# Gabisanth/MaximumAreaCoverageOptimization.jl

Measured on AMD Instinct MI355X. Metric: MADS objective evals/sec (N UAVs × M fire cells), 1/2/4/8 MI355X, higher is better.
Workload: dtype f64

## Files before the change

### maximumareacoverageoptimization.jl_amd/csrc/k_prep.h

```cpp
#pragma once

#include <hip/hip_runtime.h>
#include <stdint.h>

#include "predicate.h"
#include "k_common.h"

#pragma clang fp contract(off)

namespace mac {


struct PenArgs {
    const double* rmax;
    const double* prev;
    const double* dlimT;
    const double* dlim;
    double tan_half_fov;
};

__device__ __forceinline__ double pen_threshold(const PenArgs& pa, int i)
{
    if (!pa.prev) return 0.0;
    return pa.dlimT ? pa.dlimT[i] : dlim_threshold(pa.dlim[i]);
// ... 69 lines not shown
struct CandSrc {
    const double* cands;
    int ldc;
    const uint32_t* keysP;
    const float* keysT;
    int ldk;
    const double* xinc;
    const int* rp;
    const int* cp;
    uint64_t state;
    int64_t b;
    int k0;
    int np;
    const MadsState* mst;
    const int16_t* ltri;
    double delta;
    int route_five;
    __device__ __forceinline__ bool resolve(bool any_poll = false)
    {
        if (!mst) return true;
        const int e = mst->ell;
        if (e < 0 || (!any_poll && mst->skip)) return false;
        b = (int64_t)1 << e;
        return true;
    }
    __host__ __device__ __forceinline__ int polled(int N) const { return np ? np : 3 * N; }
    __device__ __forceinline__ double entry(int n, int r, int c) const
    {
        if (ltri) return r < c ? 0.0 : delta * (double)ltri[(int64_t)r * (r + 1) / 2 + c];
        return ltmads_entry(state, n, b, r, c);
    }
    __device__ __forceinline__ double get_full(int kl, int v, int N) const
    {
        if (cands) return cands[(int64_t)kl * ldc + v];
        const int n = 3 * N;
        const int k = kl + k0;
        const int kk = k < n ? k : k - n;
        const double d = entry(n, rp[v], cp[kk]);
        return k < n ? xinc[v] + d : xinc[v] - d;
    }
    __device__ __forceinline__ double get(int kl, int v, int N) const
    {
        if (cands) return cands[(int64_t)kl * ldc + v];
        const int n = polled(N);
        const int k = kl + k0;
        const int kk = k < n ? k : k - n;
        const bool held = v >= n;
        const double xv = xinc[v];
        const double d = entry(n, rp[held ? 0 : v], cp[kk]);
        const double moved = k < n ? xv + d : xv - d;
        return held ? xv : moved;
    }
};

#ifndef MAC_PREP_C
#define MAC_PREP_C 8
#endif
constexpr int kPrepC = MAC_PREP_C;
constexpr int kPrepU = 512;

static_assert(kPrepC % 4 == 0 && 32 % kPrepC == 0 && kPrepC <= 64,
              "MAC_PREP_C must divide 32 and be a multiple of 4");
__host__ __device__ inline int keys_ld(int K) { return (K + 31) & ~31; }

struct PrepArgs {
    CandSrc src;
    int N, K;
    PenArgs pa;
    double penalty;
    double* vp;
    int pair;
    int nchain;
    int skip_failed;
    int xbase;
    int4* prec;
    Grid g;
    uint32_t* keysP;
    float* keysT;
    int ldk;
    double4* pd;
    uint8_t* dead8;
    MadsState* mst_w;
    unsigned long long* feas;
    int* lreset;
    const uint8_t* mask8;
};

template <int NC, class Cand>
__device__ __forceinline__ uint32_t prep_masked(const uint8_t* mask8, int K, Cand cand)
{
    uint32_t m = 0u;
    if (mask8) {
#pragma unroll
        for (int c = 0; c < NC; ++c) {
            const int k = cand(c);
            if (k < K && mask8[k] == 0) m |= 1u << c;
        }
    }
    return m;
}

constexpr int kPrepCX = 6;

constexpr uint32_t kKeyEsc = 0x200u << 22;
__device__ __forceinline__ bool key_int(double v, double b, double lim, int& d)
{
    const double f = v - b;
    if (!(f >= -lim && f <= lim)) return false;
    d = (int)f;
    return (double)d == f && __builtin_bit_cast(uint64_t, b + (double)d) == __builtin_bit_cast(uint64_t, v);
}
__device__ __forceinline__ uint32_t key_pack(int dx, int dy, int dr)
{
    return ((uint32_t)dx & 0x7FFu) | (((uint32_t)dy & 0x7FFu) << 11) | (((uint32_t)dr & 0x3FFu) << 22);
}
__device__ __forceinline__ void key_unpack(uint32_t p, float& x, float& y, float& r)
{
    x = (float)((int)(p << 21) >> 21);
    y = (float)((int)(p << 10) >> 21);
    r = (float)((int)p >> 22);
}

__device__ __forceinline__ bool partial_range(double a, double b, double m, double g0, double invS,
                                              int n, int& lo, int& hi)
{
    const double ulo = (a - g0) * invS;
    const double uhi = (b - g0) * invS;
    const double err = (m + __builtin_fabs(g0)) * invS * 1e-14 + 1e-9;
    const double flo = __builtin_floor(ulo - err);
    const double fhi = __builtin_floor(uhi + err);
    if (!(flo == flo) || !(fhi == fhi)) { lo = 0; hi = n - 1; return true; }
    if (fhi < 0.0 || flo > (double)(n - 1)) return false;
    lo = flo < 0.0 ? 0 : (int)flo;
    hi = fhi > (double)(n - 1) ? n - 1 : (int)fhi;
    return true;
}

__host__ __device__ inline int range_shift(int n)
{
    int s = 0;
    while (((n - 1) >> s) > 0xFFFE) ++s;
    return s;
}
__device__ __forceinline__ uint32_t range_pack(bool any, int lo, int hi, int s)
{
    return any ? (uint32_t)(lo >> s) | ((uint32_t)(hi >> s) << 16) : 0xFFFFu;
}
__device__ __forceinline__ void range_unpack(uint32_t lo16, uint32_t hi16, int s, int n, int& lo, int& hi)
{
    lo = (int)(lo16 << s);
    hi = min((int)(((hi16 + 1) << s) - 1), n - 1);
}

#ifdef MAC_DIAG
__device__ uint64_t g_diag_prep[64 * 16];
#define MAC_PREP_STAMP_T(q, t) if (threadIdx.x == (t) && cw < 64 && (q) < 16) g_diag_prep[16 * cw + (q)] = __builtin_amdgcn_s_memrealtime()
#else
#define MAC_PREP_STAMP_T(q, t)
#endif
#define MAC_PREP_STAMP(q) MAC_PREP_STAMP_T(q, 0)

__device__ __forceinline__ void lds_barrier()
{
    asm volatile("s_waitcnt lgkmcnt(0)\n\ts_barrier" ::: "memory");
}

template <int PC>
struct PrepLds {
    double term[PC][kPrepU + 2];
    int wbad[kPrepU / kWave][PC];
    uint32_t wbadm[kPrepU / kWave];
    int wrej[kPrepU / kWave];
    double dred[kPrepU / kWave][4];
};

template <bool kMat, int PC>
__device__ __forceinline__ void prep_block(const PrepArgs& a, int cw, unsigned char* lds)
{
    constexpr int NC = PC;
    PrepLds<NC>& L = *reinterpret_cast<PrepLds<NC>*>(lds);
    auto& term = L.term;
    auto& wbad = L.wbad;
    auto& wbadm = L.wbadm;
    auto& wrej = L.wrej;
    auto& dred = L.dred;
    const int N = a.N, K = a.K;
    const int u = threadIdx.x, lane = u & (kWave - 1), wid = u / kWave;
    const int k0 = cw * PC;
    const int np = a.src.polled(N);
    auto cand = [&](int c) { return a.pair ? (c < 4 ? 4 * cw + c : np + 4 * cw + c - 4) : k0 + c; };
    const bool obj = a.vp != nullptr;
    const PenArgs& pa = a.pa;
    MAC_PREP_STAMP(0);
    double acc = 0.0;
    bool bad = false;
    uint32_t mdead = 0u;
    if constexpr (!kMat) mdead = prep_masked<NC>(obj ? a.mask8 : nullptr, K, cand);
    const bool masked = !kMat && a.mask8 != nullptr;
    const bool excl = obj && (pa.prev || masked) && (a.prec || a.pd) && a.skip_failed && N <= kPrepU;
    double dmx = -__builtin_inf(), dmy = -__builtin_inf(), dmr = -__builtin_inf();
    double dml = -__builtin_inf();
    uint32_t dead = 0u;
    for (int ib = 0; ib < N; ib += kPrepU) {
        const int nb = min(kPrepU, N - ib);
        const int i = ib + u;
        const bool iv = u < nb;
        const int ii = min(i, N - 1);
        double v[NC][3];
        if (!kMat && PC == 8 && a.pair) {
#pragma unroll
            for (int c = 0; c < 4; ++c) {
                const int col = 4 * cw + c;
#pragma unroll
                for (int q = 0; q < 3; ++q) {
                    const int vv = q * N + ii;
                    if (q == 2 && 2 * N >= np) {
                        v[c][q] = v[c + 4][q] = a.src.xinc[vv];
                        continue;
                    }
                    const double d = a.src.entry(np, a.src.rp[vv], a.src.cp[col]);
                    v[c][q] = a.src.xinc[vv] + d;
                    v[c + 4][q] = a.src.xinc[vv] - d;
                }
            }
        } else {
#pragma unroll
            for (int c = 0; c < NC; ++c) {
                const int k = min(cand(c), K - 1);
#pragma unroll
                for (int q = 0; q < 3; ++q) {
                    if constexpr (kMat) v[c][q] = a.src.cands[(int64_t)k * a.src.ldc + q * N + ii];
                    else v[c][q] = a.src.get(k, q * N + ii, N);
                }
            }
        }
        double base[3] = {0.0, 0.0, 0.0};
        if (a.keysP) {
#pragma unroll
            for (int q = 0; q < 3; ++q) {
                if constexpr (kMat) base[q] = a.src.cands[q * N + ii];
                else base[q] = a.src.get(0, q * N + ii, N);
            }
        }
        if (obj) {
            const double x1 = pa.prev ? pa.prev[ii] : 0.0, y1 = pa.prev ? pa.prev[N + ii] : 0.0;
            const double z1 = pa.prev ? pa.prev[2 * N + ii] / pa.tan_half_fov : 0.0;
            const double rm = pa.rmax ? pa.rmax[ii] : 0.0;
            const double T3 = pen_threshold(pa, ii);
            uint32_t wdead = 0u;
#pragma unroll
            for (int c = 0; c < NC; ++c) {
                const double R2 = v[c][2];
                double t = pa.rmax ? __builtin_fabs(R2 - rm) : 0.0;
                if (pa.prev) {
                    const double z2 = R2 / pa.tan_half_fov;
                    const double ddx = x1 - v[c][0], ddy = y1 - v[c][1], ddz = z1 - z2;
                    const double sq = ddx * ddx + ddy * ddy + ddz * ddz;
                    if (sq > T3) t = -1.0;
                }
                term[c][u] = t;
                const uint64_t neg = __ballot(iv && t < 0.0);
                if (lane == 0) wbad[wid][c] = neg != 0;
                wdead |= (neg != 0 ? 1u : 0u) << c;
            }
            if (lane == 0) wbadm[wid] = wdead;
            if (a.mst_w) {
                bool rej = true;
                if (iv) {
                    const double bb = (double)a.src.b;
                    rej = diag_rejects(a.src.xinc[ii], bb, x1, 0, pa.tan_half_fov, T3) &&
                          diag_rejects(a.src.xinc[N + ii], bb, y1, 1, pa.tan_half_fov, T3) &&
                          (2 * N >= np ||
                           diag_rejects(a.src.xinc[2 * N + ii], bb, pa.prev[2 * N + ii], 2, pa.tan_half_fov, T3));
                }
                const uint64_t keep = __ballot(!rej);
                if (lane == 0) wrej[wid] = keep == 0;
            }
            MAC_PREP_STAMP(1 + 3 * (ib / kPrepU));
            lds_barrier();
            if (excl) {
                dead = mdead;
#pragma unroll
                for (int w = 0; w < kPrepU / kWave; ++w) dead |= wbadm[w];
                if (a.mst_w) {
                    bool rej = true;
#pragma unroll
                    for (int w = 0; w < kPrepU / kWave; ++w) rej = rej && wrej[w] != 0;
                    if (cw == 0 && u == 0) a.mst_w->skip = rej ? 1 : 0;
                    if (rej) return;
                }
            }
            if (u < NC) {
#pragma unroll
                for (int w = 0; w < kPrepU / kWave; ++w) bad |= wbad[w][u] != 0;
                if constexpr (!kMat) bad |= ((mdead >> u) & 1u) != 0;
                if (!bad) {
                    __builtin_amdgcn_s_setprio(3);
                    constexpr int kB = 3;
                    const double2* row2 = reinterpret_cast<const double2*>(&term[u][0]);
                    const int nfull = nb / (2 * kB);
                    auto batch = [&](double2 (&buf)[kB], int bt) {
                        const int at = (bt < nfull ? bt : nfull - 1) * kB;
#pragma unroll
                        for (int j = 0; j < kB; ++j) buf[j] = row2[at + j];
                    };
                    auto add = [&](const double2 (&buf)[kB]) {
#pragma unroll
                        for (int j = 0; j < kB; ++j) {
                            acc += buf[j].x;
                            acc += buf[j].y;
                        }
                    };
                    if (nfull > 0) {
                        double2 A[kB], B[kB];
                        batch(A, 0);
#pragma unroll 1
                        for (int bt = 0; bt < nfull; bt += 2) {
                            batch(B, bt + 1);
                            __builtin_amdgcn_sched_barrier(0);
                            add(A);
                            if (bt + 1 >= nfull) break;
                            batch(A, bt + 2);
                            __builtin_amdgcn_sched_barrier(0);
                            add(B);
                        }
                    }
                    for (int q = nfull * 2 * kB; q < nb; ++q) acc += term[u][q];
                    __builtin_amdgcn_s_setprio(0);
                }
            }
            MAC_PREP_STAMP(2 + 3 * (ib / kPrepU));
        }
        if (a.pd && a.keysP && iv) {
#pragma unroll
            for (int c = 0; c < NC; ++c) {
                const double x = v[c][0], y = v[c][1], r = v[c][2];
                if (cand(c) < K && !((dead >> c) & 1u) && r > 0.0 && __builtin_isfinite(x) &&
                    __builtin_isfinite(y)) {
                    double ex = __builtin_fabs(x - base[0]), ey = __builtin_fabs(y - base[1]), er = r - base[2];
                    double el = base[2] - r;
                    if (!(ex <= kDblMax)) ex = __builtin_inf();
                    if (!(ey <= kDblMax)) ey = __builtin_inf();
                    if (!(er == er)) er = __builtin_inf();
                    if (!(el == el)) el = __builtin_inf();
                    dmx = fmax(dmx, ex);
                    dmy = fmax(dmy, ey);
                    dmr = fmax(dmr, er);
                    dml = fmax(dml, el);
                }
            }
        }
        if (a.pd && ib + kPrepU >= N) {
#pragma unroll
            for (int o = 32; o >= 1; o >>= 1) {
                dmx = fmax(dmx, __shfl_xor(dmx, o, kWave));
                dmy = fmax(dmy, __shfl_xor(dmy, o, kWave));
                dmr = fmax(dmr, __shfl_xor(dmr, o, kWave));
                dml = fmax(dml, __shfl_xor(dml, o, kWave));
            }
            if (lane == 0) {
                dred[wid][0] = dmx;
                dred[wid][1] = dmy;
                dred[wid][2] = dmr;
                dred[wid][3] = dml;
            }
        }
        if ((a.prec || a.keysP) && iv) {
            double xa = __builtin_inf(), xb = -__builtin_inf(), ya = __builtin_inf(), yb = -__builtin_inf();
            double xm = 0.0, ym = 0.0, est = 0.0;
            bool any = false;
#pragma unroll
            for (int c = 0; c < NC; ++c) {
                if (!a.prec) break;
                const double x = v[c][0], y = v[c][1], r = v[c][2];
                if (cand(c) < K && !((dead >> c) & 1u) && r > 0.0 && __builtin_isfinite(x) &&
                    __builtin_isfinite(y)) {
                    any = true;
                    xa = fmin(xa, x - r);
                    xb = fmax(xb, x + r);
                    ya = fmin(ya, y - r);
                    yb = fmax(yb, y + r);
                    xm = fmax(xm, __builtin_fabs(x) + r);
                    ym = fmax(ym, __builtin_fabs(y) + r);
                    const double e = 2.0 * r * a.g.invS + 1.0;
                    est += e * e;
                }
            }
            bool kb = false;
            if (a.keysP) {
                uint32_t pk[NC];
#pragma unroll
                for (int c = 0; c < NC; ++c) {
                    int dx = 0, dy = 0, dr = 0;
                    const bool packs = key_int(v[c][0], base[0], 1023.0, dx) &&
                                       key_int(v[c][1], base[1], 1023.0, dy) &&
                                       key_int(v[c][2], base[2], 511.0, dr);
                    pk[c] = packs ? key_pack(dx, dy, dr) : kKeyEsc;
                    if (!packs) {
#pragma unroll
                        for (int q = 0; q < 3; ++q) {
                            const float f = (float)(v[c][q] - base[q]);
                            kb |= !((dead >> c) & 1u) && __builtin_bit_cast(uint64_t, base[q] + (double)f) != __builtin_bit_cast(uint64_t, v[c][q]);
                            a.keysT[(int64_t)(q * N + i) * a.ldk + cand(c)] = f;
                        }
                    }
                }
                uint32_t* const krow = a.keysP + (int64_t)i * a.ldk;
#pragma unroll
                for (int h = 0; h < PC / 4; ++h)
                    *reinterpret_cast<uint4*>(krow + cand(4 * h)) =
                        make_uint4(pk[4 * h], pk[4 * h + 1], pk[4 * h + 2], pk[4 * h + 3]);
            }
            if (a.prec) {
                int x0 = 0, x1 = -1, y0 = 0, y1 = -1;
                any = any && partial_range(xa, xb, xm, a.g.gx0, a.g.invS, a.g.nTx, x0, x1) &&
                      partial_range(ya, yb, ym, a.g.gy0, a.g.invS, a.g.nTy, y0, y1);
                a.prec[(int64_t)cw * N + i] =
                    make_int4((int)range_pack(any, x0, x1, range_shift(a.g.nTx)),
                              (int)range_pack(any, y0, y1, range_shift(a.g.nTy)),
                              __builtin_bit_cast(int, (float)est), kb ? 1 : 0);
            }
        }
        MAC_PREP_STAMP(3 + 3 * (ib / kPrepU));
        if (obj && ib + kPrepU < N) lds_barrier();
    }
    if (obj && u < NC && cand(u) < K) {
        a.vp[cand(u)] = bad ? __builtin_inf() : acc * a.penalty;
        if (a.dead8) a.dead8[cand(u)] = excl && bad ? 1 : 0;
    }
    if (obj && a.feas && wid == 0) {
        const uint64_t ok = __ballot(u < NC && cand(u) < K && !bad);
        if (lane == 0 && ok) atomicAdd(a.feas, (unsigned long long)__popcll(ok));
    }
    if (a.pd) {
        lds_barrier();
        if (u == 0) {
            double4 m = make_double4(dred[0][0], dred[0][1], dred[0][2], dred[0][3]);
            for (int q = 1; q < kPrepU / kWave; ++q) {
                m.x = fmax(m.x, dred[q][0]);
                m.y = fmax(m.y, dred[q][1]);
                m.z = fmax(m.z, dred[q][2]);
                m.w = fmax(m.w, dred[q][3]);
            }
            a.pd[cw] = m;
        }
    }
}

template <bool kGen>
__device__ __forceinline__ void prep_block_x(const PrepArgs& a, int cw, unsigned char* lds)
{
    constexpr int PC = kPrepCX, NC = kGen ? kPrepCX : kPrepCX + 1, NW = kPrepU / kWave;
    PrepLds<kPrepCX + 1>& L = *reinterpret_cast<PrepLds<kPrepCX + 1>*>(lds);
    auto& term = L.term;
    auto& wbad = L.wbad;
    auto& wbadm = L.wbadm;
    auto& wrej = L.wrej;
    auto& dred = L.dred;
    const int N = a.N, K = a.K;
    const int u = threadIdx.x, lane = u & (kWave - 1), wid = u / kWave;
    const bool fw = wid == NW;
    const int k0 = cw * PC;
    const int n3 = 3 * N;
    auto cand = [&](int c) {
        if constexpr (kGen) return c < 3 ? 3 * cw + c : n3 + 3 * cw + c - 3;
        else return c < PC ? k0 + c : a.xbase + cw;
    };
    const bool obj = a.vp != nullptr;
    const PenArgs& pa = a.pa;
    uint32_t mdead = 0u;
    if constexpr (kGen) mdead = prep_masked<NC>(obj ? a.mask8 : nullptr, K, cand);
    const bool masked = kGen && a.mask8 != nullptr;
    const bool excl = obj && (pa.prev || masked) && a.skip_failed;
    const bool iv = !fw && u < N;
    const int ii = min(u, N - 1);
    MAC_PREP_STAMP(0);
    double v[NC][3];
    double base[3] = {0.0, 0.0, 0.0};
    if (!fw) {
        if constexpr (kGen) {
#pragma unroll
            for (int q = 0; q < 3; ++q) {
                const int vv = q * N + ii;
                const int rv = a.src.rp[vv];
                const double xv = a.src.xinc[vv];
#pragma unroll
                for (int c = 0; c < 3; ++c) {
                    const double d = a.src.entry(n3, rv, a.src.cp[3 * cw + c]);
                    v[c][q] = xv + d;
                    v[c + 3][q] = xv - d;
                }
                base[q] = xv + a.src.entry(n3, rv, a.src.cp[0]);
            }
        } else {
#pragma unroll
            for (int c = 0; c < NC; ++c) {
                const int k = min(cand(c), K - 1);
#pragma unroll
                for (int q = 0; q < 3; ++q) v[c][q] = a.src.cands[(int64_t)k * a.src.ldc + q * N + ii];
            }
#pragma unroll
            for (int q = 0; q < 3; ++q) base[q] = a.src.cands[q * N + ii];
        }
        if (obj) {
            const double x1 = pa.prev ? pa.prev[ii] : 0.0, y1 = pa.prev ? pa.prev[N + ii] : 0.0;
            const double z1 = pa.prev ? pa.prev[2 * N + ii] / pa.tan_half_fov : 0.0;
            const double rm = pa.rmax ? pa.rmax[ii] : 0.0;
            const double T3 = pen_threshold(pa, ii);
            uint32_t wdead = 0u;
#pragma unroll
            for (int c = 0; c < NC; ++c) {
                const double R2 = v[c][2];
                double t = pa.rmax ? __builtin_fabs(R2 - rm) : 0.0;
                if (pa.prev) {
                    const double z2 = R2 / pa.tan_half_fov;
                    const double ddx = x1 - v[c][0], ddy = y1 - v[c][1], ddz = z1 - z2;
                    const double sq = ddx * ddx + ddy * ddy + ddz * ddz;
                    if (sq > T3) t = -1.0;
                }
                term[c][u] = t;
                const uint64_t neg = __ballot(iv && t < 0.0);
                if (lane == 0) wbad[wid][c] = neg != 0;
                wdead |= (neg != 0 ? 1u : 0u) << c;
            }
            if (lane == 0) wbadm[wid] = wdead;
            if (a.mst_w) {
                bool rej = true;
                if (iv) {
                    const double bb = (double)a.src.b;
                    rej = diag_rejects(a.src.xinc[ii], bb, x1, 0, pa.tan_half_fov, T3) &&
                          diag_rejects(a.src.xinc[N + ii], bb, y1, 1, pa.tan_half_fov, T3) &&
                          diag_rejects(a.src.xinc[2 * N + ii], bb, pa.prev[2 * N + ii], 2, pa.tan_half_fov, T3);
                }
                const uint64_t keep = __ballot(!rej);
                if (lane == 0) wrej[wid] = keep == 0;
            }
        }
    }
    MAC_PREP_STAMP(1);
    uint32_t dead = 0u;
    if (obj) {
        lds_barrier();
        if (excl) {
            dead = mdead;
#pragma unroll
            for (int w = 0; w < NW; ++w) dead |= wbadm[w];
            if (a.mst_w) {
                bool rej = true;
#pragma unroll
                for (int w = 0; w < NW; ++w) rej = rej && wrej[w] != 0;
                if (cw == 0 && u == 0) a.mst_w->skip = rej ? 1 : 0;
                if (rej) return;
            }
        }
    }
    MAC_PREP_STAMP(2);
    if (fw) {
        bool bad = false;
        double acc = 0.0;
        if (obj && lane < NC) {
#pragma unroll
            for (int w = 0; w < NW; ++w) bad |= wbad[w][lane] != 0;
            if constexpr (kGen) bad |= ((mdead >> lane) & 1u) != 0;
            if (!bad) {
                constexpr int kB = 6;
                const double2* row2 = reinterpret_cast<const double2*>(&term[lane][0]);
                const int nfull = N / (2 * kB);
                __builtin_amdgcn_s_setprio(3);
                auto batch = [&](double2 (&buf)[kB], int bt) {
                    const int at = (bt < nfull ? bt : nfull - 1) * kB;
#pragma unroll
                    for (int j = 0; j < kB; ++j) buf[j] = row2[at + j];
                };
                auto add = [&](const double2 (&buf)[kB]) {
#pragma unroll
                    for (int j = 0; j < kB; ++j) {
                        acc += buf[j].x;
                        acc += buf[j].y;
                    }
                };
                if (nfull > 0) {
                    double2 A[kB], B[kB];
                    batch(A, 0);
#pragma unroll 1
                    for (int bt = 0; bt < nfull; bt += 2) {
                        batch(B, bt + 1);
                        __builtin_amdgcn_sched_barrier(0);
                        add(A);
                        if (bt + 1 >= nfull) break;
                        batch(A, bt + 2);
                        __builtin_amdgcn_sched_barrier(0);
                        add(B);
                    }
                }
                for (int q = nfull * 2 * kB; q < N; ++q) acc += term[lane][q];
                __builtin_amdgcn_s_setprio(0);
            }
            MAC_PREP_STAMP_T(3, kPrepU);
            if (cand(lane) < K) {
                a.vp[cand(lane)] = bad ? __builtin_inf() : acc * a.penalty;
                if (a.dead8) a.dead8[cand(lane)] = excl && bad ? 1 : 0;
            }
        }
        if (obj && a.feas) {
            const uint64_t ok = __ballot(lane < NC && cand(lane) < K && !bad);
            if (lane == 0 && ok) atomicAdd(a.feas, (unsigned long long)__popcll(ok));
        }
    } else {
        double dmx = -__builtin_inf(), dmy = -__builtin_inf(), dmr = -__builtin_inf(), dml = -__builtin_inf();
        uint32_t pk[NC];
        bool kb = false;
#pragma unroll
        for (int c = 0; c < NC; ++c) {
            const double x = v[c][0], y = v[c][1], r = v[c][2];
            int dx = 0, dy = 0, dr = 0;
            const bool packs = key_int(x, base[0], 1023.0, dx) && key_int(y, base[1], 1023.0, dy) &&
                               key_int(r, base[2], 511.0, dr);
            pk[c] = packs ? key_pack(dx, dy, dr) : kKeyEsc;
            if (!packs && iv && cand(c) < K) {
#pragma unroll
                for (int q = 0; q < 3; ++q) {
                    const float f = (float)(v[c][q] - base[q]);
                    if constexpr (kGen)
                        kb |= !((dead >> c) & 1u) &&
                              __builtin_bit_cast(uint64_t, base[q] + (double)f) != __builtin_bit_cast(uint64_t, v[c][q]);
                    a.keysT[(int64_t)(q * N + u) * a.ldk + cand(c)] = f;
                }
            }
            if (a.pd && iv && cand(c) < K && !((dead >> c) & 1u) && r > 0.0 && __builtin_isfinite(x) &&
                __builtin_isfinite(y)) {
                double ex = __builtin_fabs(x - base[0]), ey = __builtin_fabs(y - base[1]), er = r - base[2];
                double el = base[2] - r;
                if (!(ex <= kDblMax)) ex = __builtin_inf();
                if (!(ey <= kDblMax)) ey = __builtin_inf();
                if (!(er == er)) er = __builtin_inf();
                if (!(el == el)) el = __builtin_inf();
                dmx = fmax(dmx, ex);
                dmy = fmax(dmy, ey);
                dmr = fmax(dmr, er);
                dml = fmax(dml, el);
            }
        }
        if (iv) {
            uint32_t* const krow = a.keysP + (int64_t)u * a.ldk;
            if constexpr (kGen) {
#pragma unroll
                for (int c = 0; c < NC; ++c) krow[cand(c)] = pk[c];
            } else {
                static_assert(PC % 2 == 0, "an even candidate count");
#pragma unroll
                for (int h = 0; h < PC / 2; ++h)
                    *reinterpret_cast<uint2*>(krow + k0 + 2 * h) = make_uint2(pk[2 * h], pk[2 * h + 1]);
                if (cand(PC) < K) krow[cand(PC)] = pk[PC];
            }
        }
        if (kGen && a.prec && iv) {
            double xa = __builtin_inf(), xb = -__builtin_inf(), ya = __builtin_inf(), yb = -__builtin_inf();
            double xm = 0.0, ym = 0.0, est = 0.0;
            bool any = false;
#pragma unroll
            for (int c = 0; c < NC; ++c) {
                const double x = v[c][0], y = v[c][1], r = v[c][2];
                if (cand(c) < K && !((dead >> c) & 1u) && r > 0.0 && __builtin_isfinite(x) &&
                    __builtin_isfinite(y)) {
                    any = true;
                    xa = fmin(xa, x - r);
                    xb = fmax(xb, x + r);
                    ya = fmin(ya, y - r);
                    yb = fmax(yb, y + r);
                    xm = fmax(xm, __builtin_fabs(x) + r);
                    ym = fmax(ym, __builtin_fabs(y) + r);
                    const double e = 2.0 * r * a.g.invS + 1.0;
                    est += e * e;
                }
            }
            int x0 = 0, x1 = -1, y0 = 0, y1 = -1;
            any = any && partial_range(xa, xb, xm, a.g.gx0, a.g.invS, a.g.nTx, x0, x1) &&
                  partial_range(ya, yb, ym, a.g.gy0, a.g.invS, a.g.nTy, y0, y1);
            a.prec[(int64_t)cw * N + u] =
                make_int4((int)range_pack(any, x0, x1, range_shift(a.g.nTx)),
                          (int)range_pack(any, y0, y1, range_shift(a.g.nTy)),
                          __builtin_bit_cast(int, (float)est), kb ? 1 : 0);
        }
        if (a.pd) {
#pragma unroll
            for (int o = 32; o >= 1; o >>= 1) {
                dmx = fmax(dmx, __shfl_xor(dmx, o, kWave));
                dmy = fmax(dmy, __shfl_xor(dmy, o, kWave));
                dmr = fmax(dmr, __shfl_xor(dmr, o, kWave));
                dml = fmax(dml, __shfl_xor(dml, o, kWave));
            }
            if (lane == 0) {
                dred[wid][0] = dmx;
                dred[wid][1] = dmy;
                dred[wid][2] = dmr;
                dred[wid][3] = dml;
            }
        }
    }
    if (a.pd) {
        lds_barrier();
        if (u == 0) {
            double4 m = make_double4(dred[0][0], dred[0][1], dred[0][2], dred[0][3]);
            for (int q = 1; q < NW; ++q) {
                m.x = fmax(m.x, dred[q][0]);
                m.y = fmax(m.y, dred[q][1]);
                m.z = fmax(m.z, dred[q][2]);
                m.w = fmax(m.w, dred[q][3]);
            }
            a.pd[cw] = m;
        }
    }
}

template <int PC, bool kX = false, bool kGen = false>
__device__ __forceinline__ void prep_body(uint64_t* ts, PrepArgs& a)
{
    ts_begin(ts);
    if (a.lreset && blockIdx.x == 0 && threadIdx.x == 0) *a.lreset = 0;
    if (!a.src.resolve(true)) {
        ts_end(ts);
        return;
    }
    const int per = (int)((gridDim.x + 7) / 8), b = (int)blockIdx.x;
    const int cw = (int)(gridDim.x % 8) == 0 ? (b % 8) * per + b / 8 : b;
    __shared__ __attribute__((aligned(16))) unsigned char lds[sizeof(PrepLds<kX ? PC + 1 : PC>)];
    if constexpr (kX) {
        prep_block_x<kGen>(a, cw, lds);
    } else if (a.src.cands) {
        prep_block<true, PC>(a, cw, lds);
    } else {
        prep_block<false, PC>(a, cw, lds);
    }
    ts_end(ts);
}

__global__ __launch_bounds__(kPrepU) __attribute__((amdgpu_waves_per_eu(4))) void prep_kernel(uint64_t* ts, PrepArgs a)
{
    prep_body<kPrepC>(ts, a);
}

template <bool kGen>
__global__ __launch_bounds__(kPrepU + kWave) __attribute__((amdgpu_waves_per_eu(6))) void prep_x_kernel(uint64_t* ts, PrepArgs a)
{
    prep_body<kPrepCX, true, kGen>(ts, a);
}

__global__ void disk_prep_kernel(CandSrc src, int N, int K, DiskRec* __restrict__ disks)
{
    const int64_t t = (int64_t)blockIdx.x * blockDim.x + threadIdx.x;
    if (t >= (int64_t)N * K) return;
    const int k = (int)(t / N), i = (int)(t % N);
    disks[t] = make_disk(src.get(k, i, N), src.get(k, N + i, N), src.get(k, 2 * N + i, N));
}

}
```

### maximumareacoverageoptimization.jl_amd/csrc/maxcover.hip

```cpp
#include <hip/hip_runtime.h>
#include <hip/hip_ext.h>
#include <dlfcn.h>
#include <sched.h>
#include <linux/futex.h>
#include <sys/syscall.h>
#include <unistd.h>
#include <hipcub/hipcub.hpp>
#include <immintrin.h>

#include <algorithm>
#include <chrono>
#include <atomic>
#include <cmath>
#include <cstdio>
#include <cstdlib>
#include <cstring>
#include <deque>
#include <mutex>
#include <new>
#include <string>
#include <type_traits>
#include <thread>
#include <vector>

// ... 1210 lines not shown
        }
    }
    const bool tiled = use_tiled(ctx, N, hc, three_n);
    if (cons) {
        L->cmask.reserve((size_t)K);
        cons_mask_enqueue(s, L->cands.as<double>(), N, K, *cons, L->cmask.as<uint8_t>());
    }
    enqueue_eval(ctx, L, s, matrix_src(L->cands.as<double>(), N), N, (int)K, tiled, d_rmax, penalty, d_prev,
                 d_dlimT, d_prev ? L->dlimraw.as<double>() : nullptr, tan_half_fov,
                 area_out ? L->area.as<double>() : nullptr,
                 want_obj ? L->obj.as<double>() : nullptr,
                 (best_obj || best_idx) ? L->best.as<double>() : nullptr, 0);
    if (cons)
        cons_argmin_enqueue(s, L->obj.as<double>(), L->cmask.as<uint8_t>(), K, 0, L->best.p, nullptr, 0);
    double* ho = staged ? (double*)L->h_io.p : nullptr;
    double* h_area = area_out ? (staged ? ho : area_out) : nullptr;
    double* h_obj = obj_out ? (staged ? ho + (area_out ? K : 0) : obj_out) : nullptr;
    double hb_local[2] = {0, 0};
    double* hb = staged ? ho + (size_t)K * ((area_out ? 1 : 0) + (obj_out ? 1 : 0)) : hb_local;
    if (h_area) HCK(hipMemcpyAsync(h_area, L->area.p, sizeof(double) * K, hipMemcpyDeviceToHost, s));
    if (h_obj) HCK(hipMemcpyAsync(h_obj, L->obj.p, sizeof(double) * K, hipMemcpyDeviceToHost, s));
    if (best_obj || best_idx) HCK(hipMemcpyAsync(hb, L->best.p, 16, hipMemcpyDeviceToHost, s));
    HCK(hipStreamSynchronize(s));
    if (staged && area_out) std::memcpy(area_out, h_area, sizeof(double) * K);
    if (staged && obj_out) std::memcpy(obj_out, h_obj, sizeof(double) * K);
    if (best_obj) *best_obj = hb[0];
    if (best_idx) *best_idx = __builtin_bit_cast(int64_t, hb[1]);
    return MAC_OK;
}


static int32_t host_eval_basis(mac_ctx* ctx, const double* x_inc, int64_t three_n, const int16_t* ltri,
                               const int32_t* rp, const int32_t* cp, double delta, const double* r_max,
                               double penalty, const double* prev, const double* d_lim,
                               double tan_half_fov, double* obj_out, double* best_obj, int64_t* best_idx)
{
    const int64_t n = three_n;
    const int64_t K = 2 * n;
    int32_t rc = check_common(ctx, three_n, K);
    if (rc) return rc;
    if (n == 0) {
        if (best_idx) *best_idx = -1;
        if (best_obj) *best_obj = INFINITY;
        return MAC_OK;
    }
    if (!x_inc || !ltri || !rp || !cp || !r_max) return fail(MAC_E_INVAL, "null argument");
    if (!std::isfinite(delta)) return fail(MAC_E_INVAL, "delta not finite");
    for (int64_t v = 0; v < n; ++v)
        if (rp[v] < 0 || rp[v] >= n || cp[v] < 0 || cp[v] >= n)
            return fail(MAC_E_INVAL, "rp / cp entry outside [0, n)");
    if (prev && !d_lim) return fail(MAC_E_INVAL, "prev given without d_lim");
    const int N = (int)(three_n / 3);
    int64_t bmax = 1;
    for (int64_t r = 0; r < n; ++r) bmax = std::max<int64_t>(bmax, std::abs((int)ltri[r * (r + 1) / 2 + r]));
    set_device(ctx);
    LaneGuard lg(ctx);
    Lane* L = lg.lane;
    hipStream_t s = L->stream;
    const size_t tri = (size_t)n * (size_t)(n + 1) / 2;
    const size_t in_bytes = sizeof(double) * n + sizeof(int32_t) * 2 * n + sizeof(int16_t) * tri;
    const size_t out_bytes = (obj_out ? sizeof(double) * K : 0) + 16;
    L->cands.reserve(in_bytes);
    L->obj.reserve(sizeof(double) * K);
    L->best.reserve(16);
    L->h_io.reserve(std::max(in_bytes, out_bytes));
    unsigned char* h = (unsigned char*)L->h_io.p;
    std::memcpy(h, x_inc, sizeof(double) * n);
    std::memcpy(h + 8 * n, rp, sizeof(int32_t) * n);
    std::memcpy(h + 12 * n, cp, sizeof(int32_t) * n);
    std::memcpy(h + 16 * n, ltri, sizeof(int16_t) * tri);
    HCK(hipMemcpyAsync(L->cands.p, h, in_bytes, hipMemcpyHostToDevice, s));
    L->rmax.reserve(sizeof(double) * N);
    HCK(hipMemcpyAsync(L->rmax.p, r_max, sizeof(double) * N, hipMemcpyHostToDevice, s));
    double* d_prev = nullptr;
    double* d_dlimT = nullptr;
    if (prev) {
        L->prev.reserve(sizeof(double) * three_n);
        L->dlim.reserve(sizeof(double) * N);
        L->dlimraw.reserve(sizeof(double) * N);
        L->h_dlim.resize(N);
        for (int i = 0; i < N; ++i) L->h_dlim[i] = dlim_threshold(d_lim[i]);
        HCK(hipMemcpyAsync(L->prev.p, prev, sizeof(double) * three_n, hipMemcpyHostToDevice, s));
        HCK(hipMemcpyAsync(L->dlim.p, L->h_dlim.data(), sizeof(double) * N, hipMemcpyHostToDevice, s));
        HCK(hipMemcpyAsync(L->dlimraw.p, d_lim, sizeof(double) * N, hipMemcpyHostToDevice, s));
        d_prev = L->prev.as<double>();
        d_dlimT = L->dlim.as<double>();
    }
    unsigned char* d = (unsigned char*)L->cands.p;
    CandSrc src{};
    src.xinc = (const double*)d;
    src.rp = (const int*)(d + 8 * n);
    src.cp = (const int*)(d + 12 * n);
    src.ltri = (const int16_t*)(d + 16 * n);
    src.delta = delta;
    src.b = bmax;
    src.k0 = 0;
    src.route_five = host_crowded_disks(x_inc, N, (double)bmax * std::fabs(delta), ctx->grid.S) > kBitsMinDisks;
    enqueue_eval(ctx, L, s, src, N, (int)K, use_tiled(ctx, N, nullptr, three_n), L->rmax.as<double>(),
                 penalty, d_prev, d_dlimT, d_prev ? L->dlimraw.as<double>() : nullptr, tan_half_fov,
                 nullptr, L->obj.as<double>(), L->best.as<double>(), 0);
    double* ho = (double*)L->h_io.p;
    double* hb = ho + (obj_out ? K : 0);
    if (obj_out) HCK(hipMemcpyAsync(ho, L->obj.p, sizeof(double) * K, hipMemcpyDeviceToHost, s));
    HCK(hipMemcpyAsync(hb, L->best.p, 16, hipMemcpyDeviceToHost, s));
    HCK(hipStreamSynchronize(s));
    if (obj_out) std::memcpy(obj_out, ho, sizeof(double) * K);
    if (best_obj) *best_obj = hb[0];
    if (best_idx) *best_idx = __builtin_bit_cast(int64_t, hb[1]);
    return MAC_OK;
}


extern "C" {

#ifdef MAC_DIAG
int32_t mac_diag_index_read(uint64_t* out, int64_t n)
{
    if (n > (int64_t)(8 * 65536)) n = 8 * 65536;
    if (hipMemcpyFromSymbol(out, HIP_SYMBOL(g_diag_index), sizeof(uint64_t) * n, 0,
                            hipMemcpyDeviceToHost) != hipSuccess)
        return MAC_E_HIP;
    return MAC_OK;
}

int32_t mac_diag_walk_read(uint64_t* out, int64_t n)
{
    if (n > (int64_t)(8 * 65536)) n = 8 * 65536;
    if (hipMemcpyFromSymbol(out, HIP_SYMBOL(g_diag_walk), sizeof(uint64_t) * n, 0,
                            hipMemcpyDeviceToHost) != hipSuccess)
        return MAC_E_HIP;
    return MAC_OK;
}

int32_t mac_diag_fiw_read(uint64_t* out, int64_t n)
{
    if (n > (int64_t)(16 * 65536)) n = 16 * 65536;
    if (hipMemcpyFromSymbol(out, HIP_SYMBOL(g_diag_fiw), sizeof(uint64_t) * n, 0,
                            hipMemcpyDeviceToHost) != hipSuccess)
        return MAC_E_HIP;
    return MAC_OK;
}

int32_t mac_diag_f2_read(uint64_t* out, int64_t n)
{
    if (n > (int64_t)(8 * 4096)) n = 8 * 4096;
    if (hipMemcpyFromSymbol(out, HIP_SYMBOL(g_diag_f2), sizeof(uint64_t) * n, 0,
                            hipMemcpyDeviceToHost) != hipSuccess)
        return MAC_E_HIP;
    return MAC_OK;
}

int32_t mac_diag_prep_read(uint64_t* out, int64_t n)
{
    if (n > 64 * 16) n = 64 * 16;
    if (hipMemcpyFromSymbol(out, HIP_SYMBOL(g_diag_prep), sizeof(uint64_t) * n, 0,
                            hipMemcpyDeviceToHost) != hipSuccess)
        return MAC_E_HIP;
    return MAC_OK;
}

int32_t mac_diag_bits_read(uint64_t* out, int64_t n)
{
    if (n > 256 * 16) n = 256 * 16;
    if (hipMemcpyFromSymbol(out, HIP_SYMBOL(g_diag_bits), sizeof(uint64_t) * n, 0,
                            hipMemcpyDeviceToHost) != hipSuccess)
        return MAC_E_HIP;
    return MAC_OK;
}

int32_t mac_diag_or_read(uint64_t* out, int64_t n)
{
    if (n > 1024 * 16) n = 1024 * 16;
    if (hipMemcpyFromSymbol(out, HIP_SYMBOL(g_diag_or), sizeof(uint64_t) * n, 0,
                            hipMemcpyDeviceToHost) != hipSuccess)
        return MAC_E_HIP;
    return MAC_OK;
}

int32_t mac_diag_stamps(mac_ctx* ctx, uint64_t* out, int64_t n, int64_t* used)
{
    if (!ctx) return MAC_E_INVAL;
    if (hipDeviceSynchronize() != hipSuccess) return MAC_E_HIP;
    std::lock_guard<std::mutex> lk(ctx->mu);
    *used = ctx->stamp_used;
    n = std::min<int64_t>(n, 2 * ctx->stamp_used);
    if (n > 0 && hipMemcpy(out, ctx->stamps.p, sizeof(uint64_t) * n, hipMemcpyDeviceToHost) != hipSuccess)
        return MAC_E_HIP;
    return MAC_OK;
}

int32_t mac_diag_read(uint64_t* out, int64_t n)
{
    if (n > (int64_t)(4 * kDiagMax)) n = 4 * kDiagMax;
    if (hipMemcpyFromSymbol(out, HIP_SYMBOL(g_diag), sizeof(uint64_t) * n, 0, hipMemcpyDeviceToHost) != hipSuccess)
        return MAC_E_HIP;
    return MAC_OK;
}
#endif

int32_t mac_diag_grid(double xmn, double xmx, double ymn, double ymx, int64_t M, int32_t tile_points,
                      double* out)
{
    if (!out || tile_points < 1) return MAC_E_INVAL;
    const Grid g = choose_grid(xmn, xmx, ymn, ymx, M, tile_points);
    out[0] = g.S;
    out[1] = g.invS;
    out[2] = (double)g.nTx;
    out[3] = (double)g.nTy;
    return MAC_OK;
}

int32_t mac_diag_tiles(double c, double r, double g0, double invS, int32_t n, int32_t* out)
{
    if (!out || n < 1) return MAC_E_INVAL;
    int lo = -1, hi = -1;
    out[0] = tile_of(c, g0, invS, n);
    out[1] = tile_span(c, r, g0, invS, n, lo, hi) ? 1 : 0;
    out[2] = lo;
    out[3] = hi;
    return MAC_OK;
}

const char* mac_last_error(void) { return g_last_error.c_str(); }

const char* mac_version(void) { return "maxcover 0.1.0 gfx950"; }

double mac_cover_threshold(double r) { return cover_threshold(r); }

int32_t mac_profile_read(mac_ctx* ctx, double* kernel_ms, int64_t* launches,
                         int64_t* candidates, int32_t* last_algo, int32_t reset)
{
    ABI_BEGIN
    if (!ctx) return fail(MAC_E_INVAL, "null context");
    set_device(ctx);
    HCK(hipDeviceSynchronize());
    std::lock_guard<std::mutex> lk(ctx->mu);
    std::vector<uint64_t> st((size_t)(2 * ctx->stamp_used));
    if (!st.empty())
        HCK(hipMemcpy(st.data(), ctx->stamps.p, sizeof(uint64_t) * st.size(), hipMemcpyDeviceToHost));
    double ms = 0.0;
    int64_t n = 0, kc = 0;
    int algo = 0;
    auto span_ms = [&](int64_t base, int64_t nwg) {
        uint64_t t0 = ~(uint64_t)0, t1 = 0;
        for (int64_t q = base; q < base + nwg; ++q) {
            t0 = std::min(t0, st[(size_t)(2 * q)]);
            t1 = std::max(t1, st[(size_t)(2 * q + 1)]);
        }
        return t1 > t0 ? (double)(t1 - t0) / kRealtimeHz * 1e3 : 0.0;
    };
    for (auto& p : ctx->prof) {
        algo = p.algo;
        int64_t a = p.a, na = p.na;
        if (p.mode) {
            int m = 0;
            HCK(hipMemcpy(&m, p.mode, sizeof(int), hipMemcpyDeviceToHost));
            algo = m == kModePoll ? MAC_ALGO_POLL : MAC_ALGO_TILED;
            if (m == kModePoll) {
                a = p.b;
                na = p.nb;
            }
        }
        if (a < 0) continue;
        ms += span_ms(a, na);
        ++n;
        kc += p.K;
    }
    if (kernel_ms) *kernel_ms = ms;
    if (launches) *launches = n;
    if (candidates) *candidates = kc;
    if (last_algo) *last_algo = algo;
    if (reset) {
        ctx->prof.clear();
        if (ctx->stamp_used) HCK(hipMemset(ctx->stamps.p, 0, sizeof(uint64_t) * 2 * ctx->stamp_used));
        ctx->stamp_used = 0;
    }
    return MAC_OK;
    ABI_END
}

int32_t mac_profile_split(mac_ctx* ctx, double* prep_ms, double* walk_ms, double* gap_ms,
                          int64_t* polls)
{
    ABI_BEGIN
    if (!ctx) return fail(MAC_E_INVAL, "null context");
    set_device(ctx);
    HCK(hipDeviceSynchronize());
    std::lock_guard<std::mutex> lk(ctx->mu);
    std::vector<uint64_t> st((size_t)(2 * ctx->stamp_used));
    if (!st.empty())
        HCK(hipMemcpy(st.data(), ctx->stamps.p, sizeof(uint64_t) * st.size(), hipMemcpyDeviceToHost));
    double a1 = 0.0, a2 = 0.0, gap = 0.0;
    int64_t n = 0;
    for (auto& p : ctx->prof) {
        if (p.c < 0 || p.f < 0) continue;
        int64_t wa = p.a, wn = p.na;
        if (p.mode) {
            int m = 0;
            HCK(hipMemcpy(&m, p.mode, sizeof(int), hipMemcpyDeviceToHost));
            if (m == kModePoll) {
                wa = p.b;
                wn = p.nb;
            }
        }
        uint64_t s0 = ~(uint64_t)0, sw = ~(uint64_t)0, ew = 0, ef = 0;
        for (int64_t q = p.c; q < p.c + p.nc; ++q) s0 = std::min(s0, st[(size_t)(2 * q)]);
        for (int64_t q = wa; wa >= 0 && q < wa + wn; ++q) {
// ... 2559 lines not shown
```

Baseline: 43.93 million.

## Replace trailing block barrier with last-wave atomic reduction; integer pd maxima

The second block-wide barrier before the per-block pd max reduction is removed. Each wave now publishes its partial maxima and increments an LDS counter, and the last wave to arrive combines the results and writes them. The single barrier is hoisted so it also covers the pd-only case. The packed, non-generated path now tracks integer deltas and skips the per-candidate double finite checks. Diagnostic stamps are also extended per wave. This relies on the ordering of LDS atomics and waitcnt, which is subtle and adds some risk in exchange for less barrier idling.

```diff
diff --git a/maximumareacoverageoptimization.jl_amd/csrc/k_prep.h b/maximumareacoverageoptimization.jl_amd/csrc/k_prep.h
--- a/maximumareacoverageoptimization.jl_amd/csrc/k_prep.h
+++ b/maximumareacoverageoptimization.jl_amd/csrc/k_prep.h
@@ -245,11 +245,14 @@
     hi = min((int)(((hi16 + 1) << s) - 1), n - 1);
 }
 
+constexpr int kDiagPrepWg = 512;
 #ifdef MAC_DIAG
-__device__ uint64_t g_diag_prep[64 * 16];
-#define MAC_PREP_STAMP_T(q, t) if (threadIdx.x == (t) && cw < 64 && (q) < 16) g_diag_prep[16 * cw + (q)] = __builtin_amdgcn_s_memrealtime()
+__device__ uint64_t g_diag_prep[kDiagPrepWg * 16];
+#define MAC_PREP_STAMP_T(q, t) if (threadIdx.x == (t) && cw < kDiagPrepWg && (q) < 16) g_diag_prep[16 * cw + (q)] = __builtin_amdgcn_s_memrealtime()
+#define MAC_PREP_XSTAMP(q) if (lane == 0 && cw < kDiagPrepWg) g_diag_prep[16 * cw + (q)] = __builtin_amdgcn_s_memrealtime()
 #else
 #define MAC_PREP_STAMP_T(q, t)
+#define MAC_PREP_XSTAMP(q)
 #endif
 #define MAC_PREP_STAMP(q) MAC_PREP_STAMP_T(q, 0)
 
@@ -265,6 +268,7 @@
     uint32_t wbadm[kPrepU / kWave];
     int wrej[kPrepU / kWave];
     double dred[kPrepU / kWave][4];
+    uint32_t pdcnt;
 };
 
 template <bool kMat, int PC>
@@ -568,6 +572,7 @@
     const bool iv = !fw && u < N;
     const int ii = min(u, N - 1);
     MAC_PREP_STAMP(0);
+    if (u == 0) L.pdcnt = 0u;
     double v[NC][3];
     double base[3] = {0.0, 0.0, 0.0};
     if (!fw) {
@@ -628,12 +633,15 @@
                 const uint64_t keep = __ballot(!rej);
                 if (lane == 0) wrej[wid] = keep == 0;
             }
-        }
-    }
-    MAC_PREP_STAMP(1);
+#ifdef MAC_DIAG
+            asm volatile("s_waitcnt lgkmcnt(0)" ::: "memory");
+            MAC_PREP_XSTAMP(1 + wid);
+#endif
+        }
+    }
     uint32_t dead = 0u;
+    if (obj || a.pd) lds_barrier();
     if (obj) {
-        lds_barrier();
         if (excl) {
             dead = mdead;
 #pragma unroll
@@ -647,8 +655,8 @@
             }
         }
     }
-    MAC_PREP_STAMP(2);
     if (fw) {
+        MAC_PREP_XSTAMP(9);
         bool bad = false;
         double acc = 0.0;
         if (obj && lane < NC) {
@@ -689,7 +697,7 @@
                 for (int q = nfull * 2 * kB; q < N; ++q) acc += term[lane][q];
                 __builtin_amdgcn_s_setprio(0);
             }
-            MAC_PREP_STAMP_T(3, kPrepU);
+            MAC_PREP_XSTAMP(10);
             if (cand(lane) < K) {
                 a.vp[cand(lane)] = bad ? __builtin_inf() : acc * a.penalty;
                 if (a.dead8) a.dead8[cand(lane)] = excl && bad ? 1 : 0;
@@ -699,8 +707,10 @@
             const uint64_t ok = __ballot(lane < NC && cand(lane) < K && !bad);
             if (lane == 0 && ok) atomicAdd(a.feas, (unsigned long long)__popcll(ok));
         }
+        MAC_PREP_XSTAMP(12);
     } else {
         double dmx = -__builtin_inf(), dmy = -__builtin_inf(), dmr = -__builtin_inf(), dml = -__builtin_inf();
+        int imx = -1, imy = -1, imr = -1024, iml = -1024;
         uint32_t pk[NC];
         bool kb = false;
 #pragma unroll
@@ -720,19 +730,31 @@
                     a.keysT[(int64_t)(q * N + u) * a.ldk + cand(c)] = f;
                 }
             }
-            if (a.pd && iv && cand(c) < K && !((dead >> c) & 1u) && r > 0.0 && __builtin_isfinite(x) &&
-                __builtin_isfinite(y)) {
-                double ex = __builtin_fabs(x - base[0]), ey = __builtin_fabs(y - base[1]), er = r - base[2];
-                double el = base[2] - r;
-                if (!(ex <= kDblMax)) ex = __builtin_inf();
-                if (!(ey <= kDblMax)) ey = __builtin_inf();
-                if (!(er == er)) er = __builtin_inf();
-                if (!(el == el)) el = __builtin_inf();
-                dmx = fmax(dmx, ex);
-                dmy = fmax(dmy, ey);
-                dmr = fmax(dmr, er);
-                dml = fmax(dml, el);
-            }
+            if (a.pd && iv && cand(c) < K && !((dead >> c) & 1u) && r > 0.0) {
+                if (!kGen && packs) {
+                    imx = max(imx, abs(dx));
+                    imy = max(imy, abs(dy));
+                    imr = max(imr, dr);
+                    iml = max(iml, -dr);
+                } else if (__builtin_isfinite(x) && __builtin_isfinite(y)) {
+                    double ex = __builtin_fabs(x - base[0]), ey = __builtin_fabs(y - base[1]), er = r - base[2];
+                    double el = base[2] - r;
+                    if (!(ex <= kDblMax)) ex = __builtin_inf();
+                    if (!(ey <= kDblMax)) ey = __builtin_inf();
+                    if (!(er == er)) er = __builtin_inf();
+                    if (!(el == el)) el = __builtin_inf();
+                    dmx = fmax(dmx, ex);
+                    dmy = fmax(dmy, ey);
+                    dmr = fmax(dmr, er);
+                    dml = fmax(dml, el);
+                }
+            }
+        }
+        if (imx >= 0) {
+            dmx = fmax(dmx, (double)imx);
+            dmy = fmax(dmy, (double)imy);
+            dmr = fmax(dmr, (double)imr);
+            dml = fmax(dml, (double)iml);
         }
         if (iv) {
             uint32_t* const krow = a.keysP + (int64_t)u * a.ldk;
@@ -789,20 +811,25 @@
                 dred[wid][2] = dmr;
                 dred[wid][3] = dml;
             }
-        }
-    }
-    if (a.pd) {
-        lds_barrier();
-        if (u == 0) {
-            double4 m = make_double4(dred[0][0], dred[0][1], dred[0][2], dred[0][3]);
-            for (int q = 1; q < NW; ++q) {
-                m.x = fmax(m.x, dred[q][0]);
-                m.y = fmax(m.y, dred[q][1]);
-                m.z = fmax(m.z, dred[q][2]);
-                m.w = fmax(m.w, dred[q][3]);
-            }
-            a.pd[cw] = m;
-        }
+            asm volatile("s_waitcnt lgkmcnt(0)" ::: "memory");
+            if (lane == 0) {
+                const uint32_t before = atomicAdd(&L.pdcnt, 1u);
+                asm volatile("" ::: "memory");
+                if (before == (uint32_t)(NW - 1)) {
+                    double4 m = make_double4(dred[0][0], dred[0][1], dred[0][2], dred[0][3]);
+                    for (int q = 1; q < NW; ++q) {
+                        m.x = fmax(m.x, dred[q][0]);
+                        m.y = fmax(m.y, dred[q][1]);
+                        m.z = fmax(m.z, dred[q][2]);
+                        m.w = fmax(m.w, dred[q][3]);
+                    }
+                    a.pd[cw] = m;
+                    MAC_PREP_XSTAMP(13);
+                }
+            }
+        }
+        if (wid == 0) MAC_PREP_XSTAMP(11);
+        if (wid == NW - 1) MAC_PREP_XSTAMP(14);
     }
 }
 
diff --git a/maximumareacoverageoptimization.jl_amd/csrc/maxcover.hip b/maximumareacoverageoptimization.jl_amd/csrc/maxcover.hip
--- a/maximumareacoverageoptimization.jl_amd/csrc/maxcover.hip
+++ b/maximumareacoverageoptimization.jl_amd/csrc/maxcover.hip
@@ -1386,7 +1386,7 @@
 
 int32_t mac_diag_prep_read(uint64_t* out, int64_t n)
 {
-    if (n > 64 * 16) n = 64 * 16;
+    if (n > kDiagPrepWg * 16) n = kDiagPrepWg * 16;
     if (hipMemcpyFromSymbol(out, HIP_SYMBOL(g_diag_prep), sizeof(uint64_t) * n, 0,
                             hipMemcpyDeviceToHost) != hipSuccess)
         return MAC_E_HIP;
```

New measurement: 44.36 million (median of 5 runs). Within noise of the previous version (+1.0%).
